# chongkuiqi/S2ANet

Hardware: AMD Instinct MI355X
Metric: 1024x1024 DOTA chips/sec (R-50-FPN S2ANet inference) (higher is better)
Workload: dtype f16; 1 GPU; BASELINE configs[2]: full R-50-FPN S2ANet inference, batch 8 of 1024x1024 synthetic uint8 chips per GPU; 3 independent batches in flight on 3 HIP streams; global_batch=8, num_classes=15, weights=seeded random init of the reference architecture; odm_cls bias calibrated, nms_candidate_cap=160000, nms_candidates_dropped=0, distinct_input_batches=3, fam_cls_branch=True, hip_graph=False, batches_in_flight=3, parallelism=dp1 (one process per GPU)

## Files before the change

### s2anet_amd/csrc/conv_ops.hip

```cpp
#include <hip/hip_fp16.h>
#include <hip/hip_runtime.h>

#include <algorithm>
#include <cstdlib>
#include <type_traits>

#include "common.hpp"
#include "mfma_common.hpp"

namespace s2a {
namespace {

__global__ void k_pack_weight_frag(const _Float16* __restrict__ w, int O, int C, _Float16* __restrict__ wp,
                                   int taps = 9) {
  int64_t e = (int64_t)blockIdx.x * blockDim.x + threadIdx.x;
  int64_t total = (int64_t)O * C * taps;
  if (e >= total) return;
  const int G = O / 64;
  int j = (int)(e & 7);
  int lane = (int)((e >> 3) & 63);
  int kk = (int)((e >> 9) & 3);
  int mt = (int)((e >> 11) & 1);
  int64_t r = e >> 12;
  int g = (int)(r % G);
  int st = (int)(r / G);
  int t = st % taps, cc = st / taps;
  int och = g * 64 + mt * 32 + (lane & 31);
  int k = cc * 64 + kk * 16 + 8 * (lane >> 5) + j;
  wp[e] = w[((int64_t)och * C + k) * taps + t];
}

constexpr int kCPW = 18;

struct ConvExtra {
  _Float16* pool_out;
  const _Float16* head_w;
  const _Float16* head_b;
  _Float16* head_out;
  int store_main;
  const _Float16* tail_w;
  const _Float16* tail_b;
  const _Float16* tail_res;
  _Float16* tail_out;
  const _Float16* chain_w;
  const _Float16* chain_b;
  _Float16* chain_out;
  int chain_O;
};

template <int TAPS, int OG, int PH = 1, int SD = 1, bool TAIL = false, int HT = 0>
struct ConvCfg {
  static constexpr int kTH = (SD == 2 || HT) ? 4 : 8 * PH;
  static constexpr int kPos = (SD == 2 || HT) ? 64 : 128 * PH;
  static constexpr int kWaves = 4 * PH;
  static constexpr int kPW = SD == 2 ? 33 : kCPW;
  static constexpr int kNT = (kPos / 32) * OG / 4 / PH;
  static constexpr int kPix = TAPS == 9 ? ((kTH - 1) * SD + 3) * kPW : kPos;
  static constexpr int kDma = (kPix * 9 + 63) / 64;
  static constexpr int kPatchBytes = kDma * 1024;
  static constexpr int kOutRowB = OG * 128 + 16;
  static constexpr bool kWLds = PH == 2 && TAPS == 9;
  static constexpr int kWBuf = OG * 8192;
  static constexpr int kLoop0 = 2 * kPatchBytes + (kWLds ? 2 * kWBuf : 0);
  static constexpr int kLoop = (kWLds && OG == 1 && kPatchBytes + 9 * 8192 > kLoop0) ? kPatchBytes + 9 * 8192 : kLoop0;
  static constexpr int kLds0 = (kLoop > kPos * kOutRowB) ? kLoop : kPos * kOutRowB;
  static constexpr int kTailRowB = 528;
  static constexpr int kLds = (TAIL && kPos * kTailRowB > kLds0) ? kPos * kTailRowB : kLds0;
  static constexpr int kBiasBytes = TAIL ? 1024 : 512;
  static constexpr int kJ = (kDma + kWaves - 1) / kWaves;
};

template <int TAPS, int OG, int PH = 1, int SD = 1, bool TAIL = false, int HT = 0>
__global__ __launch_bounds__(256 * PH, PH == 1 ? 2 : 1) void k_conv_f16(const _Float16* __restrict__ x_,
                                                     const _Float16* __restrict__ wfrag,
                                                     const _Float16* __restrict__ bias,
                                                     const _Float16* __restrict__ residual_,
                                                     _Float16* __restrict__ out_, int64_t Ntot_, int C,
                                                     int H_, int W_, int Ho_, int Wo_, int cstride, int O,
                                                     int relu, unsigned x_bytes_, LevelTab lt, int res_up,
                                                     ConvExtra ex) {
  _Float16* pool_out_ = ex.pool_out;
  using T = _Float16;
  using V = f16x8;
  using Cfg = ConvCfg<TAPS, OG, PH, SD, TAIL, HT>;
  constexpr int NT = Cfg::kNT;
  static_assert(NT >= 1, "unsupported tile / group combination");
  static_assert(!HT || (TAPS == 9 && PH == 1 && SD == 1 && !TAIL), "half tiles: plain 3x3 / stride 1");
  static_assert(!TAIL || (TAPS == 9 && OG == 1 && SD == 1), "the fused 1x1 tail follows a 64-map 3x3/s1");
  constexpr int WPG = 4 / OG;
  constexpr int kThreads_ = 256 * PH;
  extern __shared__ __attribute__((aligned(16))) char smem[];
  const int tid = threadIdx.x, lane = tid & 63, wave = tid >> 6;
  const int wave4 = wave & 3, blk = wave >> 2;
  int64_t tile = xcd_remap(blockIdx.x, gridDim.x);
  const T* x = x_;
  const T* residual = residual_;
  T* out = out_;
  int64_t Ntot = Ntot_;
  int H = H_, W = W_, Ho = Ho_, Wo = Wo_;
  unsigned x_bytes = x_bytes_;
  if (TAPS == 9 && lt.n > 1) {
    int t0 = 0, p0 = 0;
#pragma unroll
    for (int i = 0; i < kMaxLevels; i++)
      if (i < lt.n && tile >= lt.tile0[i]) {
        t0 = lt.tile0[i]; p0 = lt.pix0[i]; H = lt.H[i]; W = lt.W[i];
      }
    tile -= t0;
    Ho = H; Wo = W;
    Ntot = (int64_t)lt.batch * H * W;
    x += (int64_t)p0 * C;
    out += (int64_t)p0 * O;
    if (residual) residual += (int64_t)p0 * O;
    if (pool_out_) pool_out_ += (int64_t)p0 * (O / 8);
    if (ex.head_out) ex.head_out += (int64_t)p0 * 64;
    x_bytes = (unsigned)(Ntot * C * 2);
  }
  const int64_t HWo = (int64_t)Ho * Wo, HWi = (int64_t)H * W;
  const int txn = (Wo + 15) / 16, tyn = (Ho + Cfg::kTH - 1) / Cfg::kTH;
  const int64_t bimg = TAPS == 9 ? tile / (txn * tyn) : 0;
  const int trem = TAPS == 9 ? (int)(tile % (txn * tyn)) : 0;
  const int ty0 = (trem / txn) * Cfg::kTH, tx0 = (trem % txn) * 16;
  const int64_t g0 = tile * Cfg::kPos;
  const int o0 = blockIdx.y * (64 * OG);
  const int Oloc = min(64 * OG, O - o0);
  const int CC = (C + 63) / 64, G = O / 64;
  const int qlim = C >= 64 ? 8 : C / 8;
  const unsigned row_bytes = (unsigned)C * 2;
  const __amdgpu_buffer_rsrc_t rx = __builtin_amdgcn_make_buffer_rsrc(const_cast<T*>(x), 0, (int)x_bytes, 0x00020000);

  const int wave_u = __builtin_amdgcn_readfirstlane(wave);
  unsigned pvoff[Cfg::kJ];
#pragma unroll
  for (int j = 0; j < Cfg::kJ; j++) {
    int v = (wave_u + Cfg::kWaves * j) * 64 + lane, p = v / 9, q = v % 9;
    bool in = q < qlim && p < Cfg::kPix;
    int64_t pix = 0;
    if (TAPS == 9) {
      int yy = ty0 * SD - 1 + p / Cfg::kPW, xx = tx0 * SD - 1 + p % Cfg::kPW;
      in = in && yy >= 0 && yy < H && xx >= 0 && xx < W;
      pix = bimg * HWi + (int64_t)yy * W + xx;
    } else {
      int64_t g = g0 + p;
      in = in && g < Ntot;
      int64_t bb = g / HWo, r = g % HWo;
      pix = bb * HWi + (r / Wo) * cstride * (int64_t)W + (r % Wo) * cstride;
    }
    pvoff[j] = in ? (unsigned)(pix * row_bytes + q * 16) : 0x80000000u;
  }
  T* s_bias = reinterpret_cast<T*>(smem + Cfg::kLds);
  T bias_v = (T)0.f;
  if (bias && tid < Oloc) bias_v = bias[o0 + tid];
  T tail_bias_v = (T)0.f;
  V wt[2][4];
  if constexpr (TAIL) {
    if (tid < 256) tail_bias_v = ex.tail_b[tid];
    const V* tp = reinterpret_cast<const V*>(ex.tail_w) + (int64_t)wave4 * 8 * 64 + ((lane >> 4) & 1) * 128 + (lane >> 5) * 32 + (lane & 15);
#pragma unroll
    for (int f = 0; f < 8; f++) wt[f >> 2][f & 3] = tp[((f >> 2) * 4 + (f & 1)) * 64 + ((f >> 1) & 1) * 16];
  }
  auto patch_issue = [&](int cc) {
    char* P = smem + (cc & 1) * Cfg::kPatchBytes;
#pragma unroll
    for (int j = 0; j < Cfg::kJ; j++) {
      const int i = wave_u + Cfg::kWaves * j;
      if (i < Cfg::kDma)
        __builtin_amdgcn_raw_ptr_buffer_load_lds(rx, (__attribute__((address_space(3))) void*)(P + i * 1024), 16,
                                                 (int)pvoff[j], cc * 128, 0, 0);
    }
  };

  const int grp = wave4 / WPG, sub = wave4 % WPG;
  const bool wave_active = grp * 64 < Oloc;
  const int g = min(o0 / 64 + grp, G - 1);
  const V* wf_base = reinterpret_cast<const V*>(wfrag) + lane;
  V wA[2][4], wB[2][4];
  constexpr bool M16 = (TAPS == 9 && SD == 1) || (TAPS == 1 && OG == 4);
  constexpr int NB16 = 2 * NT;
  auto load_w = [&](int s, V (&wv)[2][4]) {
    if constexpr (M16) {
      const V* p = reinterpret_cast<const V*>(wfrag) + ((int64_t)s * G + g) * 8 * 64 + ((lane >> 4) & 1) * 128 + (lane >> 5) * 32 + (lane & 15);
#pragma unroll
      for (int f = 0; f < 8; f++) wv[f >> 2][f & 3] = p[((f >> 2) * 4 + (f & 1)) * 64 + ((f >> 1) & 1) * 16];
      return;
    }
    const V* p = wf_base + ((int64_t)s * G + g) * 8 * 64;
#pragma unroll
    for (int a = 0; a < 2; a++)
#pragma unroll
      for (int kk = 0; kk < 4; kk++) wv[a][kk] = p[(a * 4 + kk) * 64];
  };
  const int lp = (TAPS == 9 && SD == 1) ? ((lane & 16) | (((lane & 15) - ((lane >> 3) & 2)) & 15)) : (lane & 31);
  int fbase[NT];
#pragma unroll
  for (int b = 0; b < NT; b++) {
    int pl = 128 * blk + 32 * (sub * NT + b) + lp;
    int pix = TAPS == 9 ? SD * ((pl >> 4) * Cfg::kPW + (pl & 15)) : pl;
    fbase[b] = pix * kRowBytes + (lane >> 5) * 16;
  }
  f32x16 acc[2][NT];
  f32x4 acc16[M16 ? 4 : 1][M16 ? NB16 : 1];
  if constexpr (M16) {
#pragma unroll
    for (int a = 0; a < 4; a++)
#pragma unroll
      for (int b = 0; b < NB16; b++)
#pragma unroll
        for (int r = 0; r < 4; r++) acc16[a][b][r] = 0.f;
  } else {
#pragma unroll
    for (int a = 0; a < 2; a++)
#pragma unroll
      for (int b = 0; b < NT; b++)
#pragma unroll
        for (int r = 0; r < 16; r++) acc[a][b][r] = 0.f;
  }
  const int kg16 = lane >> 4, i16 = lane & 15;
  const int pix16 = (i16 >= 4 && i16 < 12) ? (((i16 - 4) >> 1) * 4 + (i16 & 1))
                                           : (((i16 & 3) >> 1) * 4 + 2 + (i16 & 1) + (i16 >= 12 ? 8 : 0));
  const int t16 = 2 * sub * NT;
  const int fbase16 = (TAPS == 9 ? (8 * blk + t16) * Cfg::kPW + pix16 : 128 * blk + 16 * t16 + pix16) * kRowBytes + (kg16 & 1) * 64 + (kg16 >> 1) * 16;
  constexpr int kTile16 = (TAPS == 9 ? Cfg::kPW : 16) * kRowBytes;
  const int abase16 = (kg16 & 1) * 2048 + ((kg16 >> 1) * 32 + i16) * 16;

  auto compute = [&](const char* P, int t, const V (&wv)[2][4]) {
    if (!wave_active) return;
    const int toff = ((t / 3) * Cfg::kPW + (t % 3)) * kRowBytes;
    if constexpr (M16) {
#pragma unroll
      for (int ks = 0; ks < 2; ks++) {
        V pf[NB16];
#pragma unroll
        for (int b = 0; b < NB16; b++) pf[b] = *reinterpret_cast<const V*>(P + fbase16 + b * kTile16 + toff + ks * 32);
#pragma unroll
        for (int a = 0; a < 4; a++)
#pragma unroll
          for (int b = 0; b < NB16; b++)
            acc16[a][b] = __builtin_amdgcn_mfma_f32_16x16x32_f16(wv[(a * 2 + ks) >> 2][(a * 2 + ks) & 3], pf[b], acc16[a][b], 0, 0, 0);
      }
      return;
    }
#pragma unroll
    for (int kk = 0; kk < 4; kk++) {
      V pf[NT];
#pragma unroll
      for (int b = 0; b < NT; b++) pf[b] = *reinterpret_cast<const V*>(P + fbase[b] + toff + kk * 32);
#pragma unroll
      for (int a = 0; a < 2; a++)
#pragma unroll
        for (int b = 0; b < NT; b++)
          acc[a][b] = __builtin_amdgcn_mfma_f32_32x32x16_f16(wv[a][kk], pf[b], acc[a][b], 0, 0, 0);
    }
  };

  constexpr bool kEarlyRes = TAIL && Cfg::kWLds;
  constexpr int NI2 = TAIL ? Cfg::kPos * 32 / kThreads_ : 1;
  unsigned off2[NI2];
  V r2[NI2];
  auto tail_res_issue = [&]() {
    const __amdgpu_buffer_rsrc_t rr = __builtin_amdgcn_make_buffer_rsrc(
        const_cast<T*>(ex.tail_res ? ex.tail_res : ex.tail_out), 0, (int)((uint64_t)Ntot * 256 * 2), 0x00020000);
#pragma unroll
    for (int i = 0; i < NI2; i++) {
      const int idx = tid + kThreads_ * i, pos = idx >> 5, col = idx & 31;
      const int64_t gp = tile_pos(tile, pos, Cfg::kTH, Ho, Wo, HWo, Ntot);
      off2[i] = gp >= 0 ? (unsigned)((gp * 256 + col * 8) * 2) : 0x80000000u;
      r2[i] = __builtin_bit_cast(V, __builtin_amdgcn_raw_buffer_load_b128(rr, (int)(ex.tail_res ? off2[i] : 0x80000000u), 0, 0));
    }
  };
  const int nstage = TAPS * CC, last = nstage - 1;
  if constexpr (Cfg::kWLds) {
    char* wb = smem + 2 * Cfg::kPatchBytes;
    const __amdgpu_buffer_rsrc_t rw = __builtin_amdgcn_make_buffer_rsrc(
        const_cast<T*>(wfrag), 0, (int)((uint64_t)O * (uint64_t)(CC * 64) * 9 * 2), 0x00020000);
    const int wbase = (o0 / 64) * 8192;
    auto w_issue = [&](int s) {
#pragma unroll
      for (int j = 0; j < OG; j++) {
        const int piece = wave_u * OG + j;
        __builtin_amdgcn_raw_ptr_buffer_load_lds(rw, (__attribute__((address_space(3))) void*)(wb + (s & 1) * Cfg::kWBuf + piece * 1024),
                                                 16, piece * 1024 + lane * 16, s * G * 8192 + wbase, 0, 0);
      }
    };
    auto compute_wl = [&](const char* P, int t, const char* Wb) {
      const int toff = ((t / 3) * Cfg::kPW + (t % 3)) * kRowBytes;
      if constexpr (M16) {
#pragma unroll
        for (int ks = 0; ks < 2; ks++) {
          V wv[4], pf[NB16];
#pragma unroll
          for (int a = 0; a < 4; a++)
            wv[a] = *reinterpret_cast<const V*>(Wb + grp * 8192 + abase16 + (a >> 1) * 4096 + ks * 1024 + (a & 1) * 256);
#pragma unroll
          for (int b = 0; b < NB16; b++)
            pf[b] = *reinterpret_cast<const V*>(P + fbase16 + b * kTile16 + toff + ks * 32);
#pragma unroll
          for (int a = 0; a < 4; a++)
#pragma unroll
            for (int b = 0; b < NB16; b++)
              acc16[a][b] = __builtin_amdgcn_mfma_f32_16x16x32_f16(wv[a], pf[b], acc16[a][b], 0, 0, 0);
        }
        return;
      }
#pragma unroll
      for (int kk = 0; kk < 4; kk++) {
        V pf[NT], wv[2];
#pragma unroll
        for (int a = 0; a < 2; a++) wv[a] = *reinterpret_cast<const V*>(Wb + (((grp * 2 + a) * 4 + kk) * 64 + lane) * 16);
#pragma unroll
        for (int b = 0; b < NT; b++) pf[b] = *reinterpret_cast<const V*>(P + fbase[b] + toff + kk * 32);
#pragma unroll
        for (int a = 0; a < 2; a++)
#pragma unroll
          for (int b = 0; b < NT; b++)
            acc[a][b] = __builtin_amdgcn_mfma_f32_32x32x16_f16(wv[a], pf[b], acc[a][b], 0, 0, 0);
      }
    };
    if (OG == 1 && CC == 1) {
      char* wall = smem + Cfg::kPatchBytes;
      patch_issue(0);
#pragma unroll
      for (int t = 0; t < 9; t++)
        __builtin_amdgcn_raw_ptr_buffer_load_lds(rw, (__attribute__((address_space(3))) void*)(wall + t * 8192 + wave_u * 1024),
                                                 16, wave_u * 1024 + lane * 16, t * G * 8192 + wbase, 0, 0);
      if (tid < 64) s_bias[tid] = bias_v;
      if constexpr (TAIL) { if (tid < 256) s_bias[64 + tid] = tail_bias_v; }
      __syncthreads();
      if constexpr (kEarlyRes) tail_res_issue();
#pragma unroll
      for (int t = 0; t < 9; t++) compute_wl(smem, t, wall + t * 8192);
      __syncthreads();
    } else {
    patch_issue(0);
    w_issue(0);
    if (tid < 64 * OG) s_bias[tid] = bias_v;
    if constexpr (TAIL) { if (tid < 256) s_bias[64 + tid] = tail_bias_v; }
    __syncthreads();
    for (int cc = 0; cc < CC; cc++) {
      const char* Pc = smem + (cc & 1) * Cfg::kPatchBytes;
#pragma unroll
      for (int t = 0; t < 9; t++) {
        const int s = cc * 9 + t;
        if (s + 1 < nstage) w_issue(s + 1);
        if (t == 0 && cc + 1 < CC) patch_issue(cc + 1);
        compute_wl(Pc, t, wb + (s & 1) * Cfg::kWBuf);
        __syncthreads();
      }
    }
    }
  } else {
  patch_issue(0);
  load_w(0, wA);
  if (tid < 64 * OG) s_bias[tid] = bias_v;
  if constexpr (TAIL) { if (tid < 256) s_bias[64 + tid] = tail_bias_v; }
  __syncthreads();
  if constexpr (TAPS == 9) {
    for (int cc = 0; cc < CC; cc++) {
      const int s0 = cc * 9;
      const char* Pc = smem + (cc & 1) * Cfg::kPatchBytes;
#define S2A_TAP(T_, WCUR, WNEXT)                                                     \
      load_w(min(s0 + (T_) + 1, last), WNEXT);                                          \
      compute(Pc, (T_), WCUR);                                                          \
      __builtin_amdgcn_sched_barrier(0);
      S2A_TAP(0, wA, wB)
      S2A_TAP(1, wB, wA)
      S2A_TAP(2, wA, wB)
      S2A_TAP(3, wB, wA)
      S2A_TAP(4, wA, wB)
      S2A_TAP(5, wB, wA)
      if (cc + 1 < CC) patch_issue(cc + 1);
      S2A_TAP(6, wA, wB)
      S2A_TAP(7, wB, wA)
      S2A_TAP(8, wA, wB)
#undef S2A_TAP
      __syncthreads();
#pragma unroll
      for (int a = 0; a < 2; a++)
#pragma unroll
        for (int kk = 0; kk < 4; kk++) wA[a][kk] = wB[a][kk];
    }
  } else {
#define S2A_STAGE(C_, WCUR, WNEXT)                                                   \
    if ((C_) + 1 < CC) patch_issue((C_) + 1);                                           \
    load_w(min((C_) + 1, last), WNEXT);                                                 \
    compute(smem + ((C_) & 1) * Cfg::kPatchBytes, 0, WCUR);                             \
    __syncthreads();
    int cc = 0;
    for (; cc + 1 < CC; cc += 2) {
      S2A_STAGE(cc, wA, wB)
      S2A_STAGE(cc + 1, wB, wA)
    }
    if (cc < CC) { S2A_STAGE(cc, wA, wB) }
#undef S2A_STAGE
  }
  }

  char* s_out = smem;
  using h2e = __attribute__((ext_vector_type(2))) _Float16;
// ... 36 lines not shown
          }
        }
    }
  };
  if (wave_active) {
    if (relu && !residual) stage_tile(std::true_type{}); else stage_tile(std::false_type{});
  }
  __syncthreads();
  if constexpr (TAIL) {
    f32x4 acc3s[4][8];
    {
#pragma unroll
      for (int a = 0; a < 4; a++)
#pragma unroll
        for (int b = 0; b < 8; b++)
#pragma unroll
          for (int r = 0; r < 4; r++) acc3s[a][b][r] = 0.f;
      const char* brow = s_out + (128 * blk + pix16) * Cfg::kOutRowB + (kg16 & 1) * 64 + (kg16 >> 1) * 16;
#pragma unroll
      for (int ks = 0; ks < 2; ks++)
#pragma unroll
        for (int bh = 0; bh < 8; bh += 4) {
          V pf[4];
#pragma unroll
          for (int b = 0; b < 4; b++) pf[b] = *reinterpret_cast<const V*>(brow + (bh + b) * 16 * Cfg::kOutRowB + ks * 32);
#pragma unroll
          for (int a = 0; a < 4; a++)
#pragma unroll
            for (int b = 0; b < 4; b++)
              acc3s[a][bh + b] = __builtin_amdgcn_mfma_f32_16x16x32_f16(wt[(a * 2 + ks) >> 2][(a * 2 + ks) & 3], pf[b], acc3s[a][bh + b], 0, 0, 0);
        }
    }
    if constexpr (!kEarlyRes) {
      const __amdgpu_buffer_rsrc_t rr = __builtin_amdgcn_make_buffer_rsrc(
          const_cast<T*>(ex.tail_res ? ex.tail_res : ex.tail_out), 0, (int)((uint64_t)Ntot * 256 * 2), 0x00020000);
#pragma unroll
      for (int i = 0; i < NI2; i++) {
        const int idx = tid + kThreads_ * i, pos = idx >> 5, col = idx & 31;
        const int64_t gp = tile_pos(tile, pos, Cfg::kTH, Ho, Wo, HWo, Ntot);
        off2[i] = gp >= 0 ? (unsigned)((gp * 256 + col * 8) * 2) : 0x80000000u;
        r2[i] = __builtin_bit_cast(V, __builtin_amdgcn_raw_buffer_load_b128(rr, (int)(ex.tail_res ? off2[i] : 0x80000000u), 0, 0));
      }
    }
    __syncthreads();
    {
      using h4 = __attribute__((ext_vector_type(4))) _Float16;
#pragma unroll
      for (int a = 0; a < 4; a++) {
        const int och = wave4 * 64 + 16 * a + 4 * kg16;
        const h4 bq = *reinterpret_cast<const h4*>(s_bias + 64 + och);
#pragma unroll
        for (int b = 0; b < 8; b++) {
          h4 v4;
#pragma unroll
          for (int e = 0; e < 4; e++) v4[e] = (_Float16)(acc3s[a][b][e] + (float)bq[e]);
          *reinterpret_cast<h4*>(s_out + (128 * blk + 16 * b + pix16) * Cfg::kTailRowB + och * 2) = v4;
        }
      }
    }
    __syncthreads();
    const int O3 = ex.chain_O, MT = max(O3 / 32, 1);
    const int nper = (Cfg::kPos / 32) * MT / Cfg::kWaves;
    const int mt = wave % MT, nt0 = (wave / MT) * nper;
    const int G3 = O3 / 64;
    V aw[16];
    if (ex.chain_w) {
      const V* cwp = reinterpret_cast<const V*>(ex.chain_w) + lane + ((mt >> 1) * 8 + (mt & 1) * 4) * 64;
#pragma unroll
      for (int c4 = 0; c4 < 4; c4++)
#pragma unroll
        for (int kk = 0; kk < 4; kk++) aw[c4 * 4 + kk] = cwp[(c4 * G3 * 8 + kk) * 64];
    }
#pragma unroll
    for (int i = 0; i < NI2; i++) {
      const int idx = tid + kThreads_ * i, pos = idx >> 5, col = idx & 31;
      V v = *reinterpret_cast<const V*>(s_out + pos * Cfg::kTailRowB + col * 16);
#pragma unroll
      for (int e = 0; e < 8; e += 2) {
        h2e p2 = {(_Float16)((float)v[e] + (float)r2[i][e]), (_Float16)((float)v[e + 1] + (float)r2[i][e + 1])};
        p2 = __builtin_elementwise_max(p2, h2e{(_Float16)0.f, (_Float16)0.f});
        v[e] = p2[0];
        v[e + 1] = p2[1];
      }
      if (off2[i] != 0x80000000u) *reinterpret_cast<V*>(reinterpret_cast<char*>(ex.tail_out) + off2[i]) = v;
      if (ex.chain_w) *reinterpret_cast<V*>(s_out + pos * Cfg::kTailRowB + col * 16) = v;
    }
    if (ex.chain_w) {
      f32x16 c2[4];
#pragma unroll
      for (int j = 0; j < 4; j++)
#pragma unroll
        for (int r = 0; r < 16; r++) c2[j][r] = 0.f;
      __syncthreads();
#pragma unroll
      for (int c4 = 0; c4 < 4; c4++)
#pragma unroll
        for (int kk = 0; kk < 4; kk++)
#pragma unroll
          for (int j = 0; j < 4; j++)
            if (j < nper) {
              const V bf = *reinterpret_cast<const V*>(s_out + (32 * (nt0 + j) + (lane & 31)) * Cfg::kTailRowB +
                                                       (c4 * 64 + kk * 16 + (lane >> 5) * 8) * 2);
              c2[j] = __builtin_amdgcn_mfma_f32_32x32x16_f16(aw[c4 * 4 + kk], bf, c2[j], 0, 0, 0);
            }
      __syncthreads();
      const int rowb = O3 * 2 + 16;
#pragma unroll
      for (int j = 0; j < 4; j++)
        if (j < nper) {
#pragma unroll
          for (int rq = 0; rq < 4; rq++) {
            using h4 = __attribute__((ext_vector_type(4))) _Float16;
            const int och = mt * 32 + 8 * rq + 4 * (lane >> 5);
            const h4 bq = *reinterpret_cast<const h4*>(ex.chain_b + och);
            h2e lo = {(_Float16)(c2[j][rq * 4] + (float)bq[0]), (_Float16)(c2[j][rq * 4 + 1] + (float)bq[1])};
            h2e hi = {(_Float16)(c2[j][rq * 4 + 2] + (float)bq[2]), (_Float16)(c2[j][rq * 4 + 3] + (float)bq[3])};
            lo = __builtin_elementwise_max(lo, h2e{(_Float16)0.f, (_Float16)0.f});
            hi = __builtin_elementwise_max(hi, h2e{(_Float16)0.f, (_Float16)0.f});
            const h4 v4 = {lo[0], lo[1], hi[0], hi[1]};
            *reinterpret_cast<h4*>(s_out + (32 * (nt0 + j) + (lane & 31)) * rowb + och * 2) = v4;
          }
        }
      __syncthreads();
      const int vpr = O3 / 8;
      for (int idx = tid; idx < Cfg::kPos * vpr; idx += kThreads_) {
        const int pos = idx / vpr, col = idx % vpr;
        const int64_t gp = tile_pos(tile, pos, Cfg::kTH, Ho, Wo, HWo, Ntot);
        if (gp >= 0)
          *reinterpret_cast<V*>(ex.chain_out + gp * O3 + col * 8) = *reinterpret_cast<const V*>(s_out + pos * rowb + col * 16);
      }
    }
    return;
  }
  constexpr int VPR = 8 * OG;
  constexpr int NI = (Cfg::kPos * VPR) / kThreads_;
  const bool relu_u = __builtin_amdgcn_readfirstlane(relu) != 0;
  if (residual) {
    const __amdgpu_buffer_rsrc_t rr = __builtin_amdgcn_make_buffer_rsrc(
        const_cast<T*>(residual), 0, (int)((uint64_t)(res_up ? Ntot / 4 : Ntot) * O * 2), 0x00020000);
    unsigned off[NI];
    V r[NI];
    const int Wr = Wo >> 1;
    const int64_t HWr = (int64_t)(Ho >> 1) * Wr;
#pragma unroll
    for (int i = 0; i < NI; i++) {
      int idx = tid + kThreads_ * i, pos = idx / VPR, col = idx % VPR;
      int64_t gp = TAPS == 9 ? tile_pos(tile, pos, Cfg::kTH, Ho, Wo, HWo, Ntot) : (g0 + pos < Ntot ? g0 + pos : -1);
      const bool ok = gp >= 0 && col * 8 < Oloc;
      off[i] = ok ? (unsigned)((gp * O + o0 + col * 8) * 2) : 0x80000000u;
      unsigned roff = off[i];
      if (res_up && ok) {
        const int64_t bb = gp / HWo, rem = gp % HWo;
        const int yy = (int)(rem / Wo), xx = (int)(rem % Wo);
        roff = (unsigned)(((bb * HWr + (int64_t)(yy >> 1) * Wr + (xx >> 1)) * O + o0 + col * 8) * 2);
      }
      r[i] = __builtin_bit_cast(V, __builtin_amdgcn_raw_buffer_load_b128(rr, (int)roff, 0, 0));
    }
#pragma unroll
    for (int i = 0; i < NI; i++) {
      int idx = tid + kThreads_ * i, pos = idx / VPR, col = idx % VPR;
      V v = *reinterpret_cast<const V*>(s_out + pos * Cfg::kOutRowB + col * 16);
#pragma unroll
      for (int e = 0; e < 8; e += 2) {
        h2e p2 = {(_Float16)((float)v[e] + (float)r[i][e]), (_Float16)((float)v[e + 1] + (float)r[i][e + 1])};
        if (relu_u) p2 = __builtin_elementwise_max(p2, h2e{(_Float16)0.f, (_Float16)0.f});
        v[e] = p2[0];
        v[e + 1] = p2[1];
// ... 394 lines not shown
    else asm volatile("s_waitcnt vmcnt(6) lgkmcnt(0)\n\ts_barrier" ::: "memory");
    __builtin_amdgcn_sched_barrier(0);
  };
  static_assert(kNarrowJ == 7 && kNarrowDma == 26, "stage_sync counts 7 pieces on waves 0-1 and 6 on waves 2-3");
  int rb = 0;
  for (int tile = t_begin; tile < t_end; tile++) {
    const Tile cur = decode(tile);
    bool issued = false;
    for (int cc = 0; cc < CC; cc++) {
      const bool more = ivalid;
      issued = more;
      const int ncc = icc, wb = rb == 0 ? 2 : rb - 1, buf = rb;
      const char* P = smem + buf * kNarrowPatch + fbase16;
      const char* Wc = s_w + cc * (9 * 2048) + lane * 16;
      V fa[3][2], fp[3][2][2];
      auto load_tap = [&](int t, V (&a)[2], V (&p)[2][2]) {
        const int toff = ((t / 3) * kCPW + (t % 3)) * kRowBytes;
#pragma unroll
        for (int ks = 0; ks < 2; ks++) {
          a[ks] = *reinterpret_cast<const V*>(Wc + (t * 2 + ks) * 1024);
          p[ks][0] = *reinterpret_cast<const V*>(P + toff + ks * 32);
          p[ks][1] = *reinterpret_cast<const V*>(P + kTile16 + toff + ks * 32);
        }
      };
      load_tap(0, fa[0], fp[0]);
      load_tap(1, fa[1], fp[1]);
#pragma unroll
      for (int t = 0; t < 9; t++) {
        if (t + 2 < 9) load_tap(t + 2, fa[(t + 2) % 3], fp[(t + 2) % 3]);
        if (t < kNarrowJ && more) piece_issue(wb, ncc, t);
#pragma unroll
        for (int ks = 0; ks < 2; ks++) {
          acc[0] = __builtin_amdgcn_mfma_f32_16x16x32_f16(fa[t % 3][ks], fp[t % 3][ks][0], acc[0], 0, 0, 0);
          acc[1] = __builtin_amdgcn_mfma_f32_16x16x32_f16(fa[t % 3][ks], fp[t % 3][ks][1], acc[1], 0, 0, 0);
        }
        __builtin_amdgcn_sched_barrier(0);
      }
      if (more) advance();
      rb = rb == 2 ? 0 : rb + 1;
      if (cc + 1 < CC) stage_sync(more);
    }
    char* so = s_out + ((tile - t_begin) & 1) * kNarrowOutBytes;
    {
      const int och = 4 * kg16;
      const h4e bq = *reinterpret_cast<const h4e*>(s_bias + och);
#pragma unroll
      for (int b = 0; b < 2; b++) {
        h2e lo = {(_Float16)(acc[b][0] + (float)bq[0]), (_Float16)(acc[b][1] + (float)bq[1])};
        h2e hi = {(_Float16)(acc[b][2] + (float)bq[2]), (_Float16)(acc[b][3] + (float)bq[3])};
        if (relu_u) {
          lo = __builtin_elementwise_max(lo, h2e{(_Float16)0.f, (_Float16)0.f});
          hi = __builtin_elementwise_max(hi, h2e{(_Float16)0.f, (_Float16)0.f});
        }
        h4e v4 = {lo[0], lo[1], hi[0], hi[1]};
#pragma unroll
        for (int e = 0; e < 4; e++)
          if (och + e >= O_used) v4[e] = (_Float16)0.f;
        *reinterpret_cast<h4e*>(so + (16 * (2 * wave + b) + pix16) * 32 + och * 2) = v4;
#pragma unroll
        for (int r = 0; r < 4; r++) acc[b][r] = 0.f;
      }
    }
    stage_sync(issued);
#pragma unroll
    for (int i = 0; i < 4; i++) {
      const int idx = tid + 256 * i, pos = idx >> 3, col = idx & 7;
      const int y = cur.ty0 + (pos >> 4), xq = cur.tx0 + (pos & 15);
      V v;
#pragma unroll
      for (int e = 0; e < 8; e++) v[e] = (_Float16)0.f;
      if (col < 2) v = *reinterpret_cast<const V*>(so + pos * 32 + col * 16);
      if (y < cur.H && xq < cur.W) *reinterpret_cast<V*>(out + (cur.base + (int64_t)y * cur.W + xq) * 64 + col * 8) = v;
    }
  }
}

}
}

using namespace s2a;

namespace s2a {
namespace {
template <int TAPS, int OG, int PH = 1, int SD = 1, bool TAIL = false, int HT = 0>
int launch_conv(const _Float16* x, const _Float16* wfrag, const _Float16* bias, const _Float16* residual,
                _Float16* out, int64_t B, int C, int H, int W, int Ho, int Wo, int cstride, int O, int relu,
                hipStream_t st, const LevelTab* levels = nullptr, int64_t level_tiles = 0, int res_up = 0,
                ConvExtra ex = ConvExtra{nullptr, nullptr, nullptr, nullptr, 1}) {
  using Cfg = ConvCfg<TAPS, OG, PH, SD, TAIL, HT>;
  const int64_t Ntot = B * (int64_t)Ho * Wo;
  int64_t tiles = TAPS == 9 ? B * ((Wo + 15) / 16) * ((Ho + Cfg::kTH - 1) / Cfg::kTH) : (Ntot + Cfg::kPos - 1) / Cfg::kPos;
  LevelTab lt = {};
  if (levels) { lt = *levels; tiles = level_tiles; }
  dim3 grid((unsigned)tiles, (unsigned)((O + 64 * OG - 1) / (64 * OG)));
  auto kern = k_conv_f16<TAPS, OG, PH, SD, TAIL, HT>;
  S2A_HIP(hipFuncSetAttribute(reinterpret_cast<const void*>(kern), hipFuncAttributeMaxDynamicSharedMemorySize, Cfg::kLds + Cfg::kBiasBytes));
  kern<<<grid, 256 * PH, Cfg::kLds + Cfg::kBiasBytes, st>>>(x, wfrag, bias, residual, out, Ntot, C, H, W, Ho, Wo, cstride, O, relu,
                                     (unsigned)((uint64_t)B * H * W * C * 2), lt, res_up, ex);
  S2A_LAUNCH_CHECK();
  return S2A_OK;
}

struct ConvForm {
  int taps, og, ph, sd, tail, ht;
  bool operator==(const ConvForm& o) const {
    return taps == o.taps && og == o.og && ph == o.ph && sd == o.sd && tail == o.tail && ht == o.ht;
  }
};

struct ConvCall {
  const _Float16 *x, *wfrag, *bias, *residual;
  _Float16* out;
  int64_t B;
  int C, H, W, Ho, Wo, cstride, O, relu;
  hipStream_t st;
  const LevelTab* levels = nullptr;
  int64_t level_tiles = 0;
  int res_up = 0;
  ConvExtra ex = ConvExtra{nullptr, nullptr, nullptr, nullptr, 1};
  template <int TAPS, int OG, int PH = 1, int SD = 1, bool TAIL = false, int HT = 0>
  int run() const {
    return launch_conv<TAPS, OG, PH, SD, TAIL, HT>(x, wfrag, bias, residual, out, B, C, H, W, Ho, Wo, cstride, O, relu, st, levels,
                                                   level_tiles, res_up, ex);
  }
  int run(const ConvForm& f) const {
#define S2A_CONV_FORM(TAPS, OG, PH, SD, TAIL, HT) \
  if (f == ConvForm{TAPS, OG, PH, SD, TAIL, HT}) return run<TAPS, OG, PH, SD, TAIL, HT>()
    S2A_CONV_FORM(9, 4, 1, 2, 0, 0);
    S2A_CONV_FORM(9, 2, 1, 2, 0, 0);
    S2A_CONV_FORM(9, 2, 2, 1, 0, 0);
    S2A_CONV_FORM(9, 1, 2, 1, 0, 0);
    S2A_CONV_FORM(9, 4, 2, 1, 0, 0);
    S2A_CONV_FORM(9, 4, 1, 1, 0, 1);
    S2A_CONV_FORM(9, 2, 1, 1, 0, 1);
    S2A_CONV_FORM(9, 4, 1, 1, 0, 0);
    S2A_CONV_FORM(9, 2, 1, 1, 0, 0);
    S2A_CONV_FORM(9, 1, 1, 1, 0, 0);
    S2A_CONV_FORM(1, 4, 1, 2, 0, 0);
    S2A_CONV_FORM(1, 4, 1, 1, 0, 0);
    S2A_CONV_FORM(1, 2, 1, 1, 0, 0);
    S2A_CONV_FORM(1, 1, 1, 1, 0, 0);
    S2A_CONV_FORM(9, 1, 2, 1, 1, 0);
    S2A_CONV_FORM(9, 1, 1, 1, 1, 0);
#undef S2A_CONV_FORM
    s2a::set_error("conv: no kernel of form <%d, %d, %d, %d, %d, %d>", f.taps, f.og, f.ph, f.sd, f.tail, f.ht);
    return S2A_EINVAL;
  }
};

inline int env_ph(const char* name, int ph) {
  const char* f = getenv(name);
  return f ? (atoi(f) == 2 ? 2 : 1) : ph;
}
inline bool env_flag(const char* name, bool on) {
  const char* f = getenv(name);
  return f ? atoi(f) != 0 : on;
}
inline int conv_og(int64_t out_channels) { return out_channels % 256 == 0 ? 4 : (out_channels % 128 == 0 ? 2 : 1); }

ConvForm conv_form_nhwc(int64_t batch, int64_t channels, int64_t height, int64_t width, int64_t out_channels, int ksize,
                        int stride) {
  const int64_t Ho = (height - 1) / stride + 1, Wo = (width - 1) / stride + 1;
  const int og = conv_og(out_channels);
  const int64_t groups = (out_channels + 64 * og - 1) / (64 * og);
  if (ksize == 3 && stride == 2) return {9, og == 4 ? 4 : 2, 1, 2, 0, 0};
  if (ksize == 3 && og < 4 && channels % 64 == 0) {
    const int64_t tiles16 = batch * ((Wo + 15) / 16) * ((Ho + 15) / 16) * groups;
    if (env_ph("S2A_CONV_PH_NARROW", tiles16 >= 256 ? 2 : 1) == 2) return {9, og, 2, 1, 0, 0};
  }
  if (ksize == 3 && og == 4 && channels % 64 == 0) {
    const int64_t tiles16 = batch * ((Wo + 15) / 16) * ((Ho + 15) / 16) * groups;
    if (env_ph("S2A_CONV_PH", tiles16 >= 512 ? 2 : 1) == 2) return {9, 4, 2, 1, 0, 0};
  }
  if (ksize == 3 && og >= 2) {
    const int64_t wgs128 = batch * ((Wo + 15) / 16) * ((Ho + 7) / 8) * groups;
    if (env_flag("S2A_CONV3_HALF", wgs128 < 256)) return {9, og, 1, 1, 0, 1};
  }
  if (ksize == 3) return {9, og, 1, 1, 0, 0};
  if (og == 4) {
    const int64_t wgs128 = (batch * Ho * Wo + 127) / 128 * groups;
    if (env_flag("S2A_CONV1_HALF", wgs128 < 256)) return {1, 4, 1, 2, 0, 0};
  }
  return {1, og, 1, 1, 0, 0};
}

ConvForm conv_form_up2(int64_t out_channels) { return {1, conv_og(out_channels), 1, 1, 0, 0}; }

ConvForm conv_form_pyramid(int64_t channels, int64_t out_channels, bool has_head) {
  int og = conv_og(out_channels);
  const char* og_env = getenv("S2A_CONV_OG");
  if (og_env && !has_head) og = std::min(og, std::max(1, atoi(og_env)));
  if (og == 3) og = 1;
  const int ph = (og == 4 && channels % 64 == 0) ? env_ph("S2A_CONV_PH", 2) : 1;
  return {9, og, ph, 1, 0, 0};
}

ConvForm conv_form_tail(int64_t batch, int64_t height, int64_t width) {
  const int64_t tiles16 = batch * ((width + 15) / 16) * ((height + 15) / 16);
  return {9, 1, env_ph("S2A_CONV_PH_NARROW", tiles16 >= 256 ? 2 : 1), 1, 1, 0};
}

int conv_nhwc_check_sizes(int64_t batch, int64_t channels, int64_t height, int64_t width, int64_t out_channels, int ksize,
                          int stride, bool has_residual) {
  S2A_CHECK_ARG(batch >= 0 && channels > 0 && out_channels > 0 && height > 0 && width > 0, "conv: bad shape");
  S2A_CHECK_ARG(ksize == 3 || ksize == 1, "conv: kernel size must be 1 or 3");
  S2A_CHECK_ARG(stride == 1 || stride == 2, "conv: stride must be 1 or 2");
  S2A_CHECK_ARG(!(ksize == 3 && stride == 2) || out_channels % 128 == 0, "conv: 3x3 stride 2 needs out_channels % 128 == 0");
  S2A_CHECK_ARG((channels % 64 == 0 || channels == 32) && out_channels % 64 == 0,
                "conv: channels must be 32 or a multiple of 64, out_channels a multiple of 64");
  const uint64_t x_bytes = (uint64_t)batch * height * width * channels * 2;
  S2A_CHECK_ARG(x_bytes < (1ull << 31) && (ksize == 1 || (height < 32000 && width < 32000)),
                "conv: input too large for 32-bit offsets");
  S2A_CHECK_ARG(!has_residual || (uint64_t)batch * ((height - 1) / stride + 1) * ((width - 1) / stride + 1) * out_channels * 2 < (1ull << 31),
                "conv: output too large for the fused residual (32-bit offsets)");
  return S2A_OK;
}
}
}

extern "C" int s2a_conv_nhwc_f16_form(int64_t batch, int64_t channels, int64_t height, int64_t width, int64_t out_channels,
                                      int ksize, int stride, int32_t form[6]) {
  if (int rc = conv_nhwc_check_sizes(batch, channels, height, width, out_channels, ksize, stride, false)) return rc;
  S2A_CHECK_ARG(form, "conv_form: NULL form");
  const ConvForm f = conv_form_nhwc(batch, channels, height, width, out_channels, ksize, stride);
  form[0] = f.taps, form[1] = f.og, form[2] = f.ph, form[3] = f.sd, form[4] = f.tail, form[5] = f.ht;
  return S2A_OK;
}

extern "C" int s2a_conv_nhwc_f16(const void* x, const void* weight_frag, const void* bias, const void* residual,
                                 void* out, int64_t batch, int64_t channels, int64_t height, int64_t width,
                                 int64_t out_channels, int ksize, int stride, int relu, s2a_stream_t stream) {
  if (int rc = conv_nhwc_check_sizes(batch, channels, height, width, out_channels, ksize, stride, residual != nullptr)) return rc;
  if (batch == 0) return S2A_OK;
  S2A_CHECK_ARG(x && weight_frag && out, "conv: NULL tensor");
  S2A_CHECK_ARG(((uintptr_t)x % 16) == 0 && ((uintptr_t)out % 16) == 0 && ((uintptr_t)weight_frag % 16) == 0 &&
                ((uintptr_t)bias % 8) == 0 && ((uintptr_t)residual % 16) == 0, "conv: tensors must be 16-byte aligned");
  const int Ho = (int)((height - 1) / stride + 1), Wo = (int)((width - 1) / stride + 1);
  const ConvCall c{(const _Float16*)x, (const _Float16*)weight_frag, (const _Float16*)bias, (const _Float16*)residual,
                   (_Float16*)out, batch, (int)channels, (int)height, (int)width, Ho, Wo, stride, (int)out_channels, relu,
                   as_stream(stream)};
  return c.run(conv_form_nhwc(batch, channels, height, width, out_channels, ksize, stride));
}

extern "C" int s2a_conv3x3_tail1x1_f16(const void* x, const void* weight_frag, const void* bias,
                                       const void* tail_weight_frag, const void* tail_bias, const void* residual,
                                       void* out, const void* chain_weight_frag, const void* chain_bias, void* chain_out,
                                       int64_t chain_channels, int64_t batch, int64_t channels, int64_t mid_channels,
                                       int64_t out_channels, int64_t height, int64_t width, s2a_stream_t stream) {
  S2A_CHECK_ARG(batch >= 0 && height > 0 && width > 0, "conv3x3_tail1x1: bad shape");
  S2A_CHECK_ARG(channels == 64 && mid_channels == 64 && out_channels == 256,
                "conv3x3_tail1x1: built for the 64 -> 64 -> 256 bottleneck tail");
  S2A_CHECK_ARG((uint64_t)batch * height * width * out_channels * 2 < (1ull << 31) && height < 32000 && width < 32000,
                "conv3x3_tail1x1: tensor too large for 32-bit offsets");
  if (batch == 0) return S2A_OK;
  S2A_CHECK_ARG(x && weight_frag && bias && tail_weight_frag && tail_bias && out, "conv3x3_tail1x1: NULL tensor");
  S2A_CHECK_ARG(((uintptr_t)x % 16) == 0 && ((uintptr_t)out % 16) == 0 && ((uintptr_t)weight_frag % 16) == 0 &&
                ((uintptr_t)tail_weight_frag % 16) == 0 && ((uintptr_t)bias % 8) == 0 && ((uintptr_t)tail_bias % 8) == 0 &&
                ((uintptr_t)residual % 16) == 0, "conv3x3_tail1x1: tensors must be 16-byte aligned");
  ConvExtra ex{};
  ex.store_main = 0;
  ex.tail_w = (const _Float16*)tail_weight_frag;
  ex.tail_b = (const _Float16*)tail_bias;
  ex.tail_res = (const _Float16*)residual;
  ex.tail_out = (_Float16*)out;
  if (chain_weight_frag || chain_bias || chain_out) {
    S2A_CHECK_ARG(chain_weight_frag && chain_bias && chain_out, "conv3x3_tail1x1: chain filter, bias and output go together");
    S2A_CHECK_ARG(chain_channels == 64 || chain_channels == 128, "conv3x3_tail1x1: the chained 1x1 has 64 or 128 maps");
    S2A_CHECK_ARG(((uintptr_t)chain_weight_frag % 16) == 0 && ((uintptr_t)chain_bias % 8) == 0 && ((uintptr_t)chain_out % 16) == 0,
                  "conv3x3_tail1x1: chain tensors must be 16-byte aligned");
    ex.chain_w = (const _Float16*)chain_weight_frag;
    ex.chain_b = (const _Float16*)chain_bias;
    ex.chain_out = (_Float16*)chain_out;
    ex.chain_O = (int)chain_channels;
  }
  const ConvCall c{(const _Float16*)x, (const _Float16*)weight_frag, (const _Float16*)bias, nullptr, (_Float16*)out, batch, 64,
                   (int)height, (int)width, (int)height, (int)width, 1, 64, 1, as_stream(stream), nullptr, 0, 0, ex};
  return c.run(conv_form_tail(batch, height, width));
}

namespace s2a {
namespace {
template <int CC, int O3>
// ... 167 lines not shown
```

Baseline: 2038 chips/s.

## Stage fused-tail conv filters in LDS slots with a single refill

Adds a WS template parameter that gives the fused-tail 3x3 conv (PH=1, 8x16 tile) a set of LDS filter slots. It preloads WS of the 9 tap weights, computes the first taps, refills the freed slots with the remaining taps, and overlaps the residual load with that refill using counted waits and barriers. The default tail form now always uses this 5-slot PH=1 variant instead of choosing PH=2 for large tile counts, and the old PH=1 tail form is removed. The aim is to cut per-stage weight reloads and barrier overhead. In exchange it uses more LDS and hand-written waitcnt logic that depends on exactly 16 residual loads being in flight.

```diff
diff --git a/s2anet_amd/csrc/conv_ops.hip b/s2anet_amd/csrc/conv_ops.hip
--- a/s2anet_amd/csrc/conv_ops.hip
+++ b/s2anet_amd/csrc/conv_ops.hip
@@ -48,7 +48,7 @@
   int chain_O;
 };
 
-template <int TAPS, int OG, int PH = 1, int SD = 1, bool TAIL = false, int HT = 0>
+template <int TAPS, int OG, int PH = 1, int SD = 1, bool TAIL = false, int HT = 0, int WS = 0>
 struct ConvCfg {
   static constexpr int kTH = (SD == 2 || HT) ? 4 : 8 * PH;
   static constexpr int kPos = (SD == 2 || HT) ? 64 : 128 * PH;
@@ -65,12 +65,13 @@
   static constexpr int kLoop = (kWLds && OG == 1 && kPatchBytes + 9 * 8192 > kLoop0) ? kPatchBytes + 9 * 8192 : kLoop0;
   static constexpr int kLds0 = (kLoop > kPos * kOutRowB) ? kLoop : kPos * kOutRowB;
   static constexpr int kTailRowB = 528;
-  static constexpr int kLds = (TAIL && kPos * kTailRowB > kLds0) ? kPos * kTailRowB : kLds0;
+  static constexpr int kLds1 = (TAIL && kPos * kTailRowB > kLds0) ? kPos * kTailRowB : kLds0;
+  static constexpr int kLds = (WS > 0 && kPatchBytes + WS * 8192 > kLds1) ? kPatchBytes + WS * 8192 : kLds1;
   static constexpr int kBiasBytes = TAIL ? 1024 : 512;
   static constexpr int kJ = (kDma + kWaves - 1) / kWaves;
 };
 
-template <int TAPS, int OG, int PH = 1, int SD = 1, bool TAIL = false, int HT = 0>
+template <int TAPS, int OG, int PH = 1, int SD = 1, bool TAIL = false, int HT = 0, int WS = 0>
 __global__ __launch_bounds__(256 * PH, PH == 1 ? 2 : 1) void k_conv_f16(const _Float16* __restrict__ x_,
                                                      const _Float16* __restrict__ wfrag,
                                                      const _Float16* __restrict__ bias,
@@ -82,11 +83,13 @@
   _Float16* pool_out_ = ex.pool_out;
   using T = _Float16;
   using V = f16x8;
-  using Cfg = ConvCfg<TAPS, OG, PH, SD, TAIL, HT>;
+  using Cfg = ConvCfg<TAPS, OG, PH, SD, TAIL, HT, WS>;
   constexpr int NT = Cfg::kNT;
   static_assert(NT >= 1, "unsupported tile / group combination");
   static_assert(!HT || (TAPS == 9 && PH == 1 && SD == 1 && !TAIL), "half tiles: plain 3x3 / stride 1");
   static_assert(!TAIL || (TAPS == 9 && OG == 1 && SD == 1), "the fused 1x1 tail follows a 64-map 3x3/s1");
+  static_assert(WS == 0 ? (!TAIL || PH == 2) : (TAIL && PH == 1 && 2 * WS >= 9 && WS < 9),
+                "filter slots: the 8 x 16 form of the fused tail, and only it; one refill");
   constexpr int WPG = 4 / OG;
   constexpr int kThreads_ = 256 * PH;
   extern __shared__ __attribute__((aligned(16))) char smem[];
@@ -253,10 +256,16 @@
     }
   };
 
-  constexpr bool kEarlyRes = TAIL && Cfg::kWLds;
+  constexpr bool kEarlyRes = TAIL && (Cfg::kWLds || WS > 0);
   constexpr int NI2 = TAIL ? Cfg::kPos * 32 / kThreads_ : 1;
   unsigned off2[NI2];
   V r2[NI2];
+  const unsigned tail_base = (unsigned)(bimg * HWo + (int64_t)ty0 * Wo + tx0);
+  auto tail_off = [&](int i) {
+    const int idx = tid + kThreads_ * i, pos = idx >> 5, col = idx & 31;
+    const bool in = ty0 + (pos >> 4) < Ho && tx0 + (pos & 15) < Wo;
+    return in ? (tail_base + (unsigned)((pos >> 4) * Wo + (pos & 15))) * 512u + (unsigned)col * 16u : 0x80000000u;
+  };
   auto tail_res_issue = [&]() {
     const __amdgpu_buffer_rsrc_t rr = __builtin_amdgcn_make_buffer_rsrc(
         const_cast<T*>(ex.tail_res ? ex.tail_res : ex.tail_out), 0, (int)((uint64_t)Ntot * 256 * 2), 0x00020000);
@@ -264,12 +273,86 @@
     for (int i = 0; i < NI2; i++) {
       const int idx = tid + kThreads_ * i, pos = idx >> 5, col = idx & 31;
       const int64_t gp = tile_pos(tile, pos, Cfg::kTH, Ho, Wo, HWo, Ntot);
-      off2[i] = gp >= 0 ? (unsigned)((gp * 256 + col * 8) * 2) : 0x80000000u;
+      off2[i] = WS > 0 ? tail_off(i) : gp >= 0 ? (unsigned)((gp * 256 + col * 8) * 2) : 0x80000000u;
       r2[i] = __builtin_bit_cast(V, __builtin_amdgcn_raw_buffer_load_b128(rr, (int)(ex.tail_res ? off2[i] : 0x80000000u), 0, 0));
     }
   };
   const int nstage = TAPS * CC, last = nstage - 1;
-  if constexpr (Cfg::kWLds) {
+  auto compute_wl = [&](const char* P, int t, const char* Wb) {
+    const int toff = ((t / 3) * Cfg::kPW + (t % 3)) * kRowBytes;
+    if constexpr (M16) {
+#pragma unroll
+      for (int ks = 0; ks < 2; ks++) {
+        V wv[4], pf[NB16];
+#pragma unroll
+        for (int a = 0; a < 4; a++)
+          wv[a] = *reinterpret_cast<const V*>(Wb + grp * 8192 + abase16 + (a >> 1) * 4096 + ks * 1024 + (a & 1) * 256);
+#pragma unroll
+        for (int b = 0; b < NB16; b++)
+          pf[b] = *reinterpret_cast<const V*>(P + fbase16 + b * kTile16 + toff + ks * 32);
+#pragma unroll
+        for (int a = 0; a < 4; a++)
+#pragma unroll
+          for (int b = 0; b < NB16; b++)
+            acc16[a][b] = __builtin_amdgcn_mfma_f32_16x16x32_f16(wv[a], pf[b], acc16[a][b], 0, 0, 0);
+      }
+      return;
+    }
+#pragma unroll
+    for (int kk = 0; kk < 4; kk++) {
+      V pf[NT], wv[2];
+#pragma unroll
+      for (int a = 0; a < 2; a++) wv[a] = *reinterpret_cast<const V*>(Wb + (((grp * 2 + a) * 4 + kk) * 64 + lane) * 16);
+#pragma unroll
+      for (int b = 0; b < NT; b++) pf[b] = *reinterpret_cast<const V*>(P + fbase[b] + toff + kk * 32);
+#pragma unroll
+      for (int a = 0; a < 2; a++)
+#pragma unroll
+        for (int b = 0; b < NT; b++)
+          acc[a][b] = __builtin_amdgcn_mfma_f32_32x32x16_f16(wv[a], pf[b], acc[a][b], 0, 0, 0);
+    }
+  };
+  if constexpr (WS > 0) {
+    constexpr int kRefill = 9 - WS;
+    char* wslot = smem + Cfg::kPatchBytes;
+    const __amdgpu_buffer_rsrc_t rw = __builtin_amdgcn_make_buffer_rsrc(
+        const_cast<T*>(wfrag), 0, (int)((uint64_t)O * (uint64_t)(CC * 64) * 9 * 2), 0x00020000);
+    const int wbase = (o0 / 64) * 8192;
+    auto tap_issue = [&](int t, int slot) {
+#pragma unroll
+      for (int j = 0; j < 2; j++) {
+        const int piece = wave_u * 2 + j;
+        __builtin_amdgcn_raw_ptr_buffer_load_lds(rw, (__attribute__((address_space(3))) void*)(wslot + slot * 8192 + piece * 1024),
+                                                 16, piece * 1024 + lane * 16, t * G * 8192 + wbase, 0, 0);
+      }
+    };
+    patch_issue(0);
+#pragma unroll
+    for (int t = 0; t < WS; t++) tap_issue(t, t);
+    if (tid < 64) s_bias[tid] = bias_v;
+    s_bias[64 + tid] = tail_bias_v;
+    __syncthreads();
+#pragma unroll
+    for (int t = 0; t < kRefill; t++) compute_wl(smem, t, wslot + t * 8192);
+    __builtin_amdgcn_sched_barrier(0);
+    asm volatile("s_waitcnt lgkmcnt(0)\n\ts_barrier" ::: "memory");
+    __builtin_amdgcn_sched_barrier(0);
+#pragma unroll
+    for (int t = 0; t < kRefill; t++) tap_issue(WS + t, t);
+    __builtin_amdgcn_sched_barrier(0);
+    tail_res_issue();
+#pragma unroll
+    for (int t = kRefill; t < WS; t++) compute_wl(smem, t, wslot + t * 8192);
+    __builtin_amdgcn_sched_barrier(0);
+    static_assert(NI2 == 16, "the counted wait below leaves the 16 residual vectors in flight");
+    asm volatile("s_waitcnt vmcnt(16) lgkmcnt(0)\n\ts_barrier" ::: "memory");
+    __builtin_amdgcn_sched_barrier(0);
+#pragma unroll
+    for (int t = 0; t < kRefill; t++) compute_wl(smem, WS + t, wslot + t * 8192);
+    __builtin_amdgcn_sched_barrier(0);
+    asm volatile("s_waitcnt lgkmcnt(0)\n\ts_barrier" ::: "memory");
+    __builtin_amdgcn_sched_barrier(0);
+  } else if constexpr (Cfg::kWLds) {
     char* wb = smem + 2 * Cfg::kPatchBytes;
     const __amdgpu_buffer_rsrc_t rw = __builtin_amdgcn_make_buffer_rsrc(
         const_cast<T*>(wfrag), 0, (int)((uint64_t)O * (uint64_t)(CC * 64) * 9 * 2), 0x00020000);
@@ -280,40 +363,6 @@
         const int piece = wave_u * OG + j;
         __builtin_amdgcn_raw_ptr_buffer_load_lds(rw, (__attribute__((address_space(3))) void*)(wb + (s & 1) * Cfg::kWBuf + piece * 1024),
                                                  16, piece * 1024 + lane * 16, s * G * 8192 + wbase, 0, 0);
-      }
-    };
-    auto compute_wl = [&](const char* P, int t, const char* Wb) {
-      const int toff = ((t / 3) * Cfg::kPW + (t % 3)) * kRowBytes;
-      if constexpr (M16) {
-#pragma unroll
-        for (int ks = 0; ks < 2; ks++) {
-          V wv[4], pf[NB16];
-#pragma unroll
-          for (int a = 0; a < 4; a++)
-            wv[a] = *reinterpret_cast<const V*>(Wb + grp * 8192 + abase16 + (a >> 1) * 4096 + ks * 1024 + (a & 1) * 256);
-#pragma unroll
-          for (int b = 0; b < NB16; b++)
-            pf[b] = *reinterpret_cast<const V*>(P + fbase16 + b * kTile16 + toff + ks * 32);
-#pragma unroll
-          for (int a = 0; a < 4; a++)
-#pragma unroll
-            for (int b = 0; b < NB16; b++)
-              acc16[a][b] = __builtin_amdgcn_mfma_f32_16x16x32_f16(wv[a], pf[b], acc16[a][b], 0, 0, 0);
-        }
-        return;
-      }
-#pragma unroll
-      for (int kk = 0; kk < 4; kk++) {
-        V pf[NT], wv[2];
-#pragma unroll
-        for (int a = 0; a < 2; a++) wv[a] = *reinterpret_cast<const V*>(Wb + (((grp * 2 + a) * 4 + kk) * 64 + lane) * 16);
-#pragma unroll
-        for (int b = 0; b < NT; b++) pf[b] = *reinterpret_cast<const V*>(P + fbase[b] + toff + kk * 32);
-#pragma unroll
-        for (int a = 0; a < 2; a++)
-#pragma unroll
-          for (int b = 0; b < NT; b++)
-            acc[a][b] = __builtin_amdgcn_mfma_f32_32x32x16_f16(wv[a], pf[b], acc[a][b], 0, 0, 0);
       }
     };
     if (OG == 1 && CC == 1) {
@@ -516,7 +565,8 @@
         v[e] = p2[0];
         v[e + 1] = p2[1];
       }
-      if (off2[i] != 0x80000000u) *reinterpret_cast<V*>(reinterpret_cast<char*>(ex.tail_out) + off2[i]) = v;
+      const unsigned o2 = WS > 0 ? tail_off(i) : off2[i];
+      if (o2 != 0x80000000u) *reinterpret_cast<V*>(reinterpret_cast<char*>(ex.tail_out) + o2) = v;
       if (ex.chain_w) *reinterpret_cast<V*>(s_out + pos * Cfg::kTailRowB + col * 16) = v;
     }
     if (ex.chain_w) {
@@ -1077,18 +1127,18 @@
 
 namespace s2a {
 namespace {
-template <int TAPS, int OG, int PH = 1, int SD = 1, bool TAIL = false, int HT = 0>
+template <int TAPS, int OG, int PH = 1, int SD = 1, bool TAIL = false, int HT = 0, int WS = 0>
 int launch_conv(const _Float16* x, const _Float16* wfrag, const _Float16* bias, const _Float16* residual,
                 _Float16* out, int64_t B, int C, int H, int W, int Ho, int Wo, int cstride, int O, int relu,
                 hipStream_t st, const LevelTab* levels = nullptr, int64_t level_tiles = 0, int res_up = 0,
                 ConvExtra ex = ConvExtra{nullptr, nullptr, nullptr, nullptr, 1}) {
-  using Cfg = ConvCfg<TAPS, OG, PH, SD, TAIL, HT>;
+  using Cfg = ConvCfg<TAPS, OG, PH, SD, TAIL, HT, WS>;
   const int64_t Ntot = B * (int64_t)Ho * Wo;
   int64_t tiles = TAPS == 9 ? B * ((Wo + 15) / 16) * ((Ho + Cfg::kTH - 1) / Cfg::kTH) : (Ntot + Cfg::kPos - 1) / Cfg::kPos;
   LevelTab lt = {};
   if (levels) { lt = *levels; tiles = level_tiles; }
   dim3 grid((unsigned)tiles, (unsigned)((O + 64 * OG - 1) / (64 * OG)));
-  auto kern = k_conv_f16<TAPS, OG, PH, SD, TAIL, HT>;
+  auto kern = k_conv_f16<TAPS, OG, PH, SD, TAIL, HT, WS>;
   S2A_HIP(hipFuncSetAttribute(reinterpret_cast<const void*>(kern), hipFuncAttributeMaxDynamicSharedMemorySize, Cfg::kLds + Cfg::kBiasBytes));
   kern<<<grid, 256 * PH, Cfg::kLds + Cfg::kBiasBytes, st>>>(x, wfrag, bias, residual, out, Ntot, C, H, W, Ho, Wo, cstride, O, relu,
                                      (unsigned)((uint64_t)B * H * W * C * 2), lt, res_up, ex);
@@ -1098,8 +1148,9 @@
 
 struct ConvForm {
   int taps, og, ph, sd, tail, ht;
+  int ws = 0;
   bool operator==(const ConvForm& o) const {
-    return taps == o.taps && og == o.og && ph == o.ph && sd == o.sd && tail == o.tail && ht == o.ht;
+    return taps == o.taps && og == o.og && ph == o.ph && sd == o.sd && tail == o.tail && ht == o.ht && ws == o.ws;
   }
 };
 
@@ -1113,9 +1164,9 @@
   int64_t level_tiles = 0;
   int res_up = 0;
   ConvExtra ex = ConvExtra{nullptr, nullptr, nullptr, nullptr, 1};
-  template <int TAPS, int OG, int PH = 1, int SD = 1, bool TAIL = false, int HT = 0>
+  template <int TAPS, int OG, int PH = 1, int SD = 1, bool TAIL = false, int HT = 0, int WS = 0>
   int run() const {
-    return launch_conv<TAPS, OG, PH, SD, TAIL, HT>(x, wfrag, bias, residual, out, B, C, H, W, Ho, Wo, cstride, O, relu, st, levels,
+    return launch_conv<TAPS, OG, PH, SD, TAIL, HT, WS>(x, wfrag, bias, residual, out, B, C, H, W, Ho, Wo, cstride, O, relu, st, levels,
                                                    level_tiles, res_up, ex);
   }
   int run(const ConvForm& f) const {
@@ -1136,9 +1187,10 @@
     S2A_CONV_FORM(1, 2, 1, 1, 0, 0);
     S2A_CONV_FORM(1, 1, 1, 1, 0, 0);
     S2A_CONV_FORM(9, 1, 2, 1, 1, 0);
-    S2A_CONV_FORM(9, 1, 1, 1, 1, 0);
 #undef S2A_CONV_FORM
-    s2a::set_error("conv: no kernel of form <%d, %d, %d, %d, %d, %d>", f.taps, f.og, f.ph, f.sd, f.tail, f.ht);
+    if (f == ConvForm{9, 1, 1, 1, 1, 0, 6}) return run<9, 1, 1, 1, true, 0, 6>();
+    if (f == ConvForm{9, 1, 1, 1, 1, 0, 5}) return run<9, 1, 1, 1, true, 0, 5>();
+    s2a::set_error("conv: no kernel of form <%d, %d, %d, %d, %d, %d, %d>", f.taps, f.og, f.ph, f.sd, f.tail, f.ht, f.ws);
     return S2A_EINVAL;
   }
 };
@@ -1190,9 +1242,13 @@
   return {9, og, ph, 1, 0, 0};
 }
 
+constexpr int kTailSlots = 5;
 ConvForm conv_form_tail(int64_t batch, int64_t height, int64_t width) {
-  const int64_t tiles16 = batch * ((width + 15) / 16) * ((height + 15) / 16);
-  return {9, 1, env_ph("S2A_CONV_PH_NARROW", tiles16 >= 256 ? 2 : 1), 1, 1, 0};
+  (void)batch, (void)height, (void)width;
+  const int ph = env_ph("S2A_CONV_PH_NARROW", 1);
+  if (ph == 2) return {9, 1, 2, 1, 1, 0};
+  const char* slots = getenv("S2A_CONV_TAIL_SLOTS");
+  return {9, 1, 1, 1, 1, 0, slots ? (atoi(slots) == 6 ? 6 : 5) : kTailSlots};
 }
 
 int conv_nhwc_check_sizes(int64_t batch, int64_t channels, int64_t height, int64_t width, int64_t out_channels, int ksize,
```

After: 2033 chips/s. No clear change (-0.3%).
